# rojas-diego/tokengeex

Measured on AMD Instinct MI355X. Metric: MB/s raw bytes encoded (and tokens/s) at 32K/64K vocab, 1/2/4/8 GPUs, higher is better.
Workload: dtype f64

## Files before the change

### tokengeex_amd/csrc/encode2.hip

```cpp
#include <hip/hip_runtime.h>
#include <stdint.h>

#include "device_common.h"
#include "kernels.h"
#include "trace_body.h"

namespace tgx {

constexpr uint32_t kNoStep2 = 0xFFu;
constexpr uint32_t kRows2Bytes = 64u * 32u * 8u;
constexpr uint64_t kHiHalf = 0xFFFFFFFF00000000ULL;

template <int U>
__device__ __forceinline__ void relax2_step(double sv, double& acc, uint32_t& bpv, uint32_t& fin, uint32_t& fhi) {
    constexpr uint64_t MU = (1ULL << U) | (1ULL << (32 + U));
    fin = sel_u32(MU, bpv, fin);
    fhi = sel_u32(MU, (uint32_t)((uint64_t)__double_as_longlong(acc) >> 32), fhi);
    const double b0 = readlane_f64(acc, (uint32_t)U), b1 = readlane_f64(acc, 32u + (uint32_t)U);
    const double best = sel_f64(kHiHalf, b1, b0);
    const double cand = best + sv;
    const uint64_t take = __builtin_amdgcn_fcmp(cand, acc, 2 ) | MU;
    acc = sel_f64(take, cand, acc);
    bpv = sel_imm_u32<U>(take, bpv);
}
// ... 104 lines not shown
            relax2_step<1>(sv[1], acc, bpv, fin, fhi);
            relax2_step<2>(sv[2], acc, bpv, fin, fhi);
            relax2_step<3>(sv[3], acc, bpv, fin, fhi);
            relax2_step<4>(sv[4], acc, bpv, fin, fhi);
            relax2_step<5>(sv[5], acc, bpv, fin, fhi);
            relax2_step<6>(sv[6], acc, bpv, fin, fhi);
            relax2_step<7>(sv[7], acc, bpv, fin, fhi);
            relax2_step<8>(sv[8], acc, bpv, fin, fhi);
            relax2_step<9>(sv[9], acc, bpv, fin, fhi);
            relax2_step<10>(sv[10], acc, bpv, fin, fhi);
            relax2_step<11>(sv[11], acc, bpv, fin, fhi);
            relax2_step<12>(sv[12], acc, bpv, fin, fhi);
            relax2_step<13>(sv[13], acc, bpv, fin, fhi);
            relax2_step<14>(sv[14], acc, bpv, fin, fhi);
            relax2_step<15>(sv[15], acc, bpv, fin, fhi);
#pragma unroll
            for (int u = 0; u < 16; ++u) sv[u] = scr[(u + 16) * 32];
            relax2_step<16>(sv[0], acc, bpv, fin, fhi);
            relax2_step<17>(sv[1], acc, bpv, fin, fhi);
            relax2_step<18>(sv[2], acc, bpv, fin, fhi);
            relax2_step<19>(sv[3], acc, bpv, fin, fhi);
            relax2_step<20>(sv[4], acc, bpv, fin, fhi);
            relax2_step<21>(sv[5], acc, bpv, fin, fhi);
            relax2_step<22>(sv[6], acc, bpv, fin, fhi);
            relax2_step<23>(sv[7], acc, bpv, fin, fhi);
            relax2_step<24>(sv[8], acc, bpv, fin, fhi);
            relax2_step<25>(sv[9], acc, bpv, fin, fhi);
            relax2_step<26>(sv[10], acc, bpv, fin, fhi);
            relax2_step<27>(sv[11], acc, bpv, fin, fhi);
            relax2_step<28>(sv[12], acc, bpv, fin, fhi);
            relax2_step<29>(sv[13], acc, bpv, fin, fhi);
            relax2_step<30>(sv[14], acc, bpv, fin, fhi);
            relax2_step<31>(sv[15], acc, bpv, fin, fhi);
        }
        __builtin_amdgcn_wave_barrier();
        const bool reached = fhi != 0xFFF00000u;

        if (live && pg >= 1u && pg <= n) {
            const uint8_t b = reached ? (uint8_t)((l - fin - 1u) & 31u) : (uint8_t)0xFF;
            __builtin_nontemporal_store(b, P.bp8 + bp8_base(beg, s) + (PERM ? bp8_perm(pg - 1u) : pg - 1u));
        }
        if (live) {
            const uint32_t left = n - p0;
            if (left < 32u) {
                if (left == l) P.status[s] = (n == 0u || reached) ? 1u : 0u;
                need_new = true;
            } else {
                p0 += 32u;
            }
        }
    }
}

template <bool PERM, bool CARRY, int K>
__global__ __launch_bounds__(256) void trace32_kernel(EncodeParams P) {
    __shared__ typename TraceRingEntry<CARRY>::type ring_all[4][kTraceRing];
    trace_body<32, PERM, false, CARRY, K>(P, ring_all[threadIdx.x >> 6]);
}

hipError_t launch_encode2(const EncodeParams& p, uint32_t num_cus, bool permuted, hipStream_t stream) {
    const uint32_t waves = 5, bpc = 2;
    const uint64_t want = (p.n_samples + 2 * waves - 1) / (2 * waves);
    const uint32_t blocks = (uint32_t)(want < (uint64_t)num_cus * bpc ? (want ? want : 1) : (uint64_t)num_cus * bpc);
    auto fn = p.dropout > 0.0 ? (permuted ? encode2_kernel<true, true> : encode2_kernel<true, false>)
                              : (permuted ? encode2_kernel<false, true> : encode2_kernel<false, false>);
    hipError_t e = hipFuncSetAttribute(reinterpret_cast<const void*>(fn), hipFuncAttributeMaxDynamicSharedMemorySize, 160 * 1024);
    if (e != hipSuccess) return e;
    hipLaunchKernelGGL(fn, dim3(blocks), dim3(64u * waves), waves * kRows2Bytes, stream, p);
    return hipGetLastError();
}
template <bool PERM, bool CARRY>
static void launch_trace32_stride(const EncodeParams& p, uint32_t blocks, hipStream_t stream) {
    switch (p.trace_stride) {
        case 1: hipLaunchKernelGGL((trace32_kernel<PERM, CARRY, 1>), dim3(blocks), dim3(256), 0, stream, p); break;
        case 2: hipLaunchKernelGGL((trace32_kernel<PERM, CARRY, 2>), dim3(blocks), dim3(256), 0, stream, p); break;
        case 3: hipLaunchKernelGGL((trace32_kernel<PERM, CARRY, 3>), dim3(blocks), dim3(256), 0, stream, p); break;
        default: hipLaunchKernelGGL((trace32_kernel<PERM, CARRY, 0>), dim3(blocks), dim3(256), 0, stream, p); break;
    }
}
hipError_t launch_trace32(const EncodeParams& p, uint32_t blocks, bool permuted, hipStream_t stream) {
    if (permuted) {
        if (p.trace_carry) launch_trace32_stride<true, true>(p, blocks, stream);
        else launch_trace32_stride<true, false>(p, blocks, stream);
    } else {
        if (p.trace_carry) launch_trace32_stride<false, true>(p, blocks, stream);
        else launch_trace32_stride<false, false>(p, blocks, stream);
    }
    return hipGetLastError();
}

}
```

### tokengeex_amd/csrc/encode_pass.cpp

```cpp
#include <hip/hip_runtime.h>

#include <algorithm>
#include <chrono>
#include <condition_variable>
#include <cstdio>
#include <cstdlib>
#include <cstring>
#include <mutex>
#include <numeric>
#include <string>
#include <thread>
#include <vector>

#include "../../include/tgx.h"
#include "api_internal.h"
#include "device_internal.h"
#include "pass_internal.h"
#include "kernels.h"
#include "encode_split.h"
#include "ids_in_place.h"
#include "trie_build.h"

using namespace tgx::host;
using namespace tgx::dev;
// ... 46 lines not shown
    std::vector<double> v2((size_t)nv + 1), w2(wvalues.size());
    v2[0] = values[0];
    if (!w2.empty()) w2[0] = wvalues[0];
    unsigned long long total = 0, run = 0;
    for (uint32_t r = 0; r < nv; r++) total += cnt[order[r]];
    std::vector<double> cov((size_t)nv + 1, 0.0);
    for (uint32_t r = 0; r < nv; r++) {
        perm[order[r]] = r + 1u;
        v2[r + 1u] = values[order[r]];
        if (!w2.empty()) w2[r + 1u] = wvalues[order[r]];
        run += cnt[order[r]];
        cov[r + 1u] = total ? (double)run / (double)total : 1.0;
    }
    cov[nv] = 1.0;
    ok = hipMemcpyAsync(d_perm, perm.data(), ((size_t)nv + 1) * 4, hipMemcpyHostToDevice, m->stream) == hipSuccess &&
         tgx::launch_rank_remap(m->d_trie8, (uint32_t)m->flat.table.size(), d_perm, m->stream) == hipSuccess &&
         hipMemcpyAsync(m->d_values, v2.data(), ((size_t)nv + 1) * 8, hipMemcpyHostToDevice, m->stream) == hipSuccess &&
         (w2.empty() || hipMemcpyAsync(m->d_wvalues, w2.data(), ((size_t)nv + 1) * 8, hipMemcpyHostToDevice, m->stream) == hipSuccess) &&
         hipStreamSynchronize(m->stream) == hipSuccess;
    if (!ok) return fail(TGX_ERR_DEVICE, "value re-rank failed: %s", hipGetErrorString(hipGetLastError()));
    m->value_coverage = std::move(cov);
    hp.mark("re-rank");
    return pass.done();
}

}

namespace tgx::dev {

tgx::EncodeParams base_encode_params(const tgx_model* m, const tgx_corpus* c, uint64_t seed) {
    tgx::EncodeParams p{};
    p.text = c->d_text;
    p.offs = c->d_offs;
    p.order = c->d_order;
    p.n_samples = c->n_samples;
    p.trie = m->d_trie;
    p.tokid = m->d_tokid;
    p.root_base = m->flat.table[0].base & ~tgx::kTerminalBit;
    p.lm = m->lm;
    p.n_slots = (uint32_t)m->flat.table.size();
    p.bp = c->d_bp;
    p.tmp = c->d_tmp;
    p.counts = c->d_counts;
    p.status = c->d_status;
    p.bp8 = reinterpret_cast<uint8_t*>(c->d_bp.get());
    p.tokhash = m->d_tokhash;
    p.tokhash_mask = m->tokhash.mask;
    p.tokhash_seed = m->tokhash.seed;
    p.err_sample = &m->d_ctrl->err;
    p.queue = &m->d_ctrl->queue;
    p.seed = seed;
    p.trace_carry = (c->n_samples && c->n_bytes / c->n_samples < 2048) ? 1u : 0u;
    p.trace_stride = tgx::kTraceStride;
    return p;
}

tgx_status check_no_path(tgx_model* m, const tgx_corpus* c) {
    unsigned long long bad = m->h_ctrl->err;
    if (bad == ~0ULL) return TGX_OK;
    if (bad & tgx::kErrCorruptBp)
        return fail(TGX_ERR_DEVICE, "internal error: corrupt back-pointer (sample or text byte %llu)",
                    (unsigned long long)(bad & ~tgx::kErrCorruptBp));
    if (bad & tgx::kErrCountMismatch)
        return fail(TGX_ERR_DEVICE, "internal error: the token count of sample %llu differs between the relaxation and the trace",
                    (unsigned long long)(bad & ~tgx::kErrCountMismatch));
    uint64_t n = c->h_offs[bad + 1] - c->h_offs[bad];
    set_error_detail(bad, n, n);
    return fail(TGX_ERR_NO_PATH, "no path to position %llu/%llu", (unsigned long long)n,
                (unsigned long long)n);
}

}

namespace {

tgx_status redo_long_matches(tgx_model* m, tgx_corpus* c, const tgx::EncodeParams& p) {
    unsigned long long n_redo = 0;
    HIP_TRY(hipMemcpyAsync(&n_redo, &m->d_ctrl->encode_redo, 8, hipMemcpyDeviceToHost, m->stream));
    HIP_TRY(hipStreamSynchronize(m->stream));
    if (n_redo > c->n_samples) return fail(TGX_ERR_DEVICE, "redo list longer than the batch");
    m->last_redo_samples = n_redo;
    if (n_redo) {
        tgx::EncodeParams q = p;
        q.order = c->d_counts;
        q.n_samples = n_redo;
        HIP_TRY(hipMemsetAsync(&m->d_ctrl->queue, 0x00, 8, m->stream));
        time_begin(m, "encode2_kernel");
        HIP_TRY(tgx::launch_encode2(q, (uint32_t)m->num_cus, true, m->stream));
        time_end(m);
    }
    return TGX_OK;
}

tgx_status scan_ids_offsets(tgx_model* m, tgx_corpus* c, tgx_result* r, const char* what, bool with_err);

struct Encode6Choice {
    int e6_bpc;
    uint32_t n_hot6;
    uint32_t pool6;
    bool cold6;
    bool e6_usable;
};
Encode6Choice choose_encode6(const tgx_model* m) {
    int e6_bpc = 2;
    if (const char* e = knob("TGX_E6_BPC")) e6_bpc = std::min(4, std::max(1, atoi(e)));
    uint32_t n_hot6 = std::min(m->n_values, tgx::encode6_max_hot(160u * 1024u / (uint32_t)e6_bpc, 0u));
// ... 102 lines not shown
    if (const char* e = long_tokens ? nullptr : knob("TGX_PPL")) {
        const int v = atoi(e);
        if (v >= 1 && v <= 4) {
            ppl = v;
            bpc = ppl >= 3 ? 1 : 2;
        }
    }
    knob_int("TGX_BPC", 1, 8, &bpc);
    const uint32_t budget = 160u * 1024u / (uint32_t)bpc;
    bool cold = false;
    int per_simd = 0;
    HIP_TRY(tgx::encode5_waves_per_simd(dropout > 0.0, false, ppl, long_tokens, compact, lean, step_ok, want_count, &per_simd));
    int waves = std::min(16, (per_simd / bpc) * 4);
    if ((ppl == 4 || ppl == 3) && bpc == 1 && hot_waves > 0) waves = std::min(waves, hot_waves);
    if (m->n_values > tgx::encode5_max_hot(long_tokens, waves, ppl, budget)) {
        cold = true;
        HIP_TRY(tgx::encode5_waves_per_simd(dropout > 0.0, true, ppl, long_tokens, compact, lean, step_ok, want_count, &per_simd));
        waves = std::min(16, (per_simd / bpc) * 4);
    }
    if (balance_waves > 0 && ppl == 4 && bpc == 1) waves = std::min(waves, balance_waves);
    waves = waves_for_units(waves, rest_n, (uint64_t)cus5 * bpc);
    knob_int("TGX_WAVES", 1, 16, &waves);
    while (waves > 1 && tgx::encode5_max_hot(long_tokens, waves, ppl, budget) < 16u) waves--;
    uint32_t n_hot = std::min(m->n_values, tgx::encode5_max_hot(long_tokens, waves, ppl, budget));
    n_hot = knob_cap_hot("TGX_E5_HOT", n_hot);
    cold = n_hot < m->n_values;
    iq.build_counts = tgx::encode5_counts(dropout > 0.0, cold, ppl, long_tokens);
    const bool in_place = want_count && tgx::ids_in_place(iq);
    const uint64_t rows_per_block = 4 * (uint64_t)waves;
    const uint32_t blocks5 = (uint32_t)std::max<uint64_t>(
        1, std::min<uint64_t>((rest_n + rows_per_block - 1) / rows_per_block, (uint64_t)cus5 * bpc));
    *out = Encode5Geometry{ppl, bpc, waves, per_simd, cold, n_hot, blocks5, compact, lean, step_ok, in_place};
    return TGX_OK;
}

tgx_status trace_rows5(tgx_model* m, tgx_corpus* c, tgx::EncodeParams& p, bool long_tokens, bool in_place, Pass& pass, tgx_result* r) {
    const uint32_t blocks_t = trace_blocks(m, c->n_samples);
    if (in_place) {
        const tgx_status st = scan_ids_offsets(m, c, r, "encode", false);
        if (st != TGX_OK) return st;
        time_begin(m, "trace_kernel");
        HIP_TRY(tgx::launch_trace_in_place(p, tgx::TraceInPlace{r->d_offs, r->d_ids}, blocks_t, m->stream));
        time_end(m);
        m->last_ids_in_place = true;
        return TGX_OK;
    }
    Stamps stamps_t;
    if (!long_tokens) stamps_t = stamps_begin(m, pass, '2', (size_t)blocks_t * 4);
    p.stamps = stamps_t.d;
    time_begin(m, long_tokens ? "trace32_kernel" : "trace_kernel");
    if (long_tokens) HIP_TRY(tgx::launch_trace32(p, blocks_t, true, m->stream));
    else HIP_TRY(tgx::launch_trace(p, blocks_t, m->stream));
    time_end(m);
    if (stamps_t.d) stamps_report(m, stamps_t, 0, "trace stamps", "window", {"setup", "loads", "hops", "append+lookups", "-"});
    p.stamps = nullptr;
    return TGX_OK;
}

tgx_status encode_rows5(tgx_model* m, tgx_corpus* c, tgx::EncodeParams& p, bool long_tokens, Pass& pass, tgx_result* r) {
    tgx_status st = ensure_value_ranks(m, c);
    if (st != TGX_OK) return st;
    m->last_redo_samples = 0;
    const Encode6Choice e6 = choose_encode6(m);
    tgx::EncodeSplit split;
    if (c->n_samples && !long_tokens && e6.e6_usable) split = split_long_samples(m, c, e6);
    const uint64_t n_long = split.n_long;
    const uint32_t corun_cus = split.corun_cus;
    Encode5Geometry g;
    if ((st = choose_encode5(m, c, p, long_tokens, n_long, corun_cus, r != nullptr, &g)) != TGX_OK) return st;
    m->last_n_hot = g.n_hot;
    if (!g.in_place) {
        if ((st = ensure_scratch(c, true)) != TGX_OK) return st;
        p.tmp = c->d_tmp;
    }
    const uint64_t rest_n = c->n_samples - n_long;
    m->last_lean_items = !g.lean ? 0u : ((rest_n ? (uint32_t)tgx::encode5_lean_items(g.cold, g.ppl, g.step_ok) : 0u) |
                                         (n_long ? (uint32_t)tgx::encode6_lean_items() << 8 : 0u));
    m->last_encode_waves_per_cu = std::min(g.bpc, g.per_simd / ((g.waves + 3) / 4)) * g.waves;
    tgx::Encode5Params q{};
    q.trie8 = m->d_trie8;
    q.trie_bytes = (uint32_t)(m->flat.table.size() * sizeof(tgx::Trie8Rec));
    q.values = m->d_values;
    q.root_base = m->root_base8;
    q.n_values = m->n_values;
    q.n_hot = g.n_hot;
    q.claim_chunk = claim_chunk_for(c->n_bytes, c->n_samples);
    if (const char* e = knob("TGX_CLAIM_CHUNK")) q.claim_chunk = (uint32_t)std::min(64, std::max(1, atoi(e)));
    m->last_long_samples = n_long;
    m->last_corun_cus = n_long ? corun_cus : 0u;
    tgx::EncodeParams p6 = p;
    tgx::Encode5Params q6 = q;
    uint32_t blocks6 = 0;
    if (n_long) {
        p6.n_samples = n_long;
        blocks6 = (uint32_t)std::min<uint64_t>((n_long + 3) / 4, (uint64_t)(corun_cus ? (int)corun_cus : m->num_cus) * (uint64_t)e6.e6_bpc);
        q6.n_hot = e6.n_hot6;
        q6.pool = e6.cold6 ? e6.pool6 : 0u;
        if (!corun_cus) {
            time_begin(m, "encode6_kernel");
            HIP_TRY(tgx::launch_encode6(p6, q6, e6.cold6, g.lean, blocks6, m->stream));
            time_end(m);
            HIP_TRY(hipMemsetAsync(&m->d_ctrl->queue, 0x00, 8, m->stream));
        } else {
            if (!m->stream2) {
                HIP_TRY(hipStreamCreateWithFlags(&m->stream2, hipStreamNonBlocking));
                HIP_TRY(hipEventCreateWithFlags(&m->ev_fork, hipEventDisableTiming));
                HIP_TRY(hipEventCreateWithFlags(&m->ev_join, hipEventDisableTiming));
// ... 113 lines not shown
    p.stamps = stamps4.d;
    time_begin(m, "encode4_kernel");
    HIP_TRY(tgx::launch_encode4(p, ppl, waves, blocks4, root, m->stream));
    time_end(m);
    if (stamps4.d) stamps_report(m, stamps4, 0, "stamps", "iteration", {"switch", "text", "walk", "relax", "store"});
    p.stamps = nullptr;
    p.order = c->d_order;
    p.n_samples = c->n_samples;
    time_begin(m, "trace_kernel");
    HIP_TRY(tgx::launch_trace(p, trace_blocks(m, c->n_samples), m->stream));
    time_end(m);
    return TGX_OK;
}

tgx_status encode_rows2(tgx_model* m, tgx_corpus* c, tgx::EncodeParams& p, bool rows2) {
    m->last_redo_samples = 0;
    if (!rows2) {
        p.redo_count = &m->d_ctrl->encode_redo;
        p.redo_list = c->d_counts;
        HIP_TRY(hipMemsetAsync(&m->d_ctrl->encode_redo, 0x00, 8, m->stream));
        time_begin(m, "encode4l_kernel");
        HIP_TRY(tgx::launch_encode4l(p, (uint32_t)m->num_cus, m->stream));
        time_end(m);
        const tgx_status rst = redo_long_matches(m, c, p);
        if (rst != TGX_OK) return rst;
    } else {
        time_begin(m, "encode2_kernel");
        HIP_TRY(tgx::launch_encode2(p, (uint32_t)m->num_cus, false, m->stream));
        time_end(m);
    }
    time_begin(m, "trace32_kernel");
    HIP_TRY(tgx::launch_trace32(p, trace_blocks(m, c->n_samples), !rows2, m->stream));
    time_end(m);
    return TGX_OK;
}

tgx_status encode_fused(tgx_model* m, tgx_corpus* c, const tgx::EncodeParams& p) {
    time_begin(m, "encode_kernel");
    HIP_TRY(tgx::launch_encode(p, grid_blocks(m, c->n_samples), m->stream));
    time_end(m);
    return TGX_OK;
}

tgx_status run_encode_kernel(tgx_model* m, tgx_corpus* c, double dropout, uint64_t seed, Pass& pass, tgx_result* r) {
    m->last_ids_in_place = false;
    tgx_status st = ensure_scratch(c, false);
    if (st != TGX_OK) return st;
    HIP_TRY(hipMemsetAsync(&m->d_ctrl->queue, 0x00, 8, m->stream));
    HIP_TRY(hipMemsetAsync(&m->d_ctrl->err, 0xFF, 8, m->stream));
    tgx::EncodeParams p = base_encode_params(m, c, seed);
    p.dropout = dropout;
    if (const char* e = knob("TGX_TRACE_CARRY")) p.trace_carry = atoi(e) ? 1u : 0u;
    if (const char* e = knob("TGX_TRACE_STRIDE")) p.trace_stride = (uint32_t)std::min(3, std::max(0, atoi(e)));
    p.flags = debug_flags();
    const char* force = knob("TGX_PATH");
    const bool use4 = m->lm <= 16 && m->scores_finite && m->d_tokhash && !(force && strcmp(force, "fused") == 0);
    const bool use2 = !use4 && m->lm <= 32 && m->scores_finite && m->d_tokhash && !(force && strcmp(force, "fused") == 0);
    const bool long_tokens = m->lm > 16;
    const bool use5 = (use4 || use2) && m->have_trie8 &&
                      !(force && (strcmp(force, "rows4") == 0 || strcmp(force, "rows2") == 0 || strcmp(force, "rows4l") == 0));
    if (debug_on())
        fprintf(stderr, "[tgx] encode: S=%llu N=%llu lm=%u path=%s slots=%zu root_base=%u values=%u\n",
                (unsigned long long)c->n_samples, (unsigned long long)c->n_bytes, p.lm, use4 ? (use5 ? "rows5" : "rows4") : (use2 ? "rows2" : "fused"),
                m->flat.table.size(), p.root_base, m->n_values);
    m->last_lean_items = 0;
    if (use5) return encode_rows5(m, c, p, long_tokens, pass, r);
    if ((st = ensure_scratch(c, true)) != TGX_OK) return st;
    p.tmp = c->d_tmp;
    if (use4) return encode_rows4(m, c, p, pass);
    if (use2) return encode_rows2(m, c, p, force && strcmp(force, "rows2") == 0);
    return encode_fused(m, c, p);
}

tgx_status scan_ids_offsets(tgx_model* m, tgx_corpus* c, tgx_result* r, const char* what, bool with_err) {
    const uint64_t S = c->n_samples;
    if (!c->d_scan_tmp) {
        if (tgx::scan_temp_bytes(S, &c->scan_tmp_bytes) != hipSuccess) return fail(TGX_ERR_DEVICE, "scan temp-size query failed");
        if (c->scan_tmp_bytes && c->d_scan_tmp.alloc(m->device, c->scan_tmp_bytes) != hipSuccess)
            return fail(TGX_ERR_DEVICE, "out of device memory (scan)");
    }
    time_begin(m, "scan_counts_kernel");
    if (tgx::launch_scan(c->d_counts, r->d_offs, S, c->d_scan_tmp, c->scan_tmp_bytes, m->stream) != hipSuccess)
        return fail(TGX_ERR_DEVICE, "scan launch failed");
    time_end(m);
    if ((with_err && hipMemcpyAsync(&m->h_ctrl->err, &m->d_ctrl->err, 8, hipMemcpyDeviceToHost, m->stream) != hipSuccess) ||
        hipMemcpyAsync(&m->h_ctrl->total_tokens, r->d_offs + S, 8, hipMemcpyDeviceToHost, m->stream) != hipSuccess ||
        hipStreamSynchronize(m->stream) != hipSuccess)
        return fail(TGX_ERR_DEVICE, "%s pass failed: %s", what, hipGetErrorString(hipGetLastError()));
    if (with_err) {
        const tgx_status st = check_no_path(m, c);
        if (st != TGX_OK) return st;
    }
    r->n_tokens = m->h_ctrl->total_tokens;
    if (r->n_tokens > c->n_bytes) return fail(TGX_ERR_DEVICE, "internal error: %s pass counted more tokens than bytes", what);
    if (r->d_ids.alloc(m->device, (size_t)r->n_tokens * 4 + 256) != hipSuccess)
        return fail(TGX_ERR_DEVICE, "out of device memory (result ids)");
    return TGX_OK;
}

}

tgx_status tgx::dev::compact_ids(tgx_model* m, tgx_corpus* c, tgx_result* r, const char* what) {
    const uint64_t S = c->n_samples;
    const tgx_status sst = scan_ids_offsets(m, c, r, what, true);
    if (sst != TGX_OK) return sst;
    tgx::CompactParams cp{};
// ... 346 lines not shown
```

### tokengeex_amd/csrc/kernels.h

```cpp
#pragma once
#include <hip/hip_runtime.h>
#include <stdint.h>

#include "decode.h"
#include "fim.h"
#include "spans.h"

namespace tgx {

constexpr uint32_t kTraceStride = 2;

struct EncodeParams {
    const uint8_t* text;
    const uint64_t* offs;
    const uint32_t* order;
    uint64_t n_samples;
    const void* trie;
    const uint32_t* tokid;
    uint32_t root_base;
    uint32_t n_slots;
    uint32_t lm;
    uint32_t* bp;
    uint32_t* tmp;
    uint32_t* counts;
    uint32_t* status;
    uint8_t* bp8;
    const void* tokhash;
    uint32_t tokhash_mask;
    uint32_t tokhash_seed;
    unsigned long long* err_sample;
    unsigned long long* queue;
    unsigned long long* redo_count;
    uint32_t* redo_list;
    double dropout;
    uint64_t seed;
    uint32_t flags;
    unsigned long long* stamps;
    uint32_t trace_carry;
    uint32_t trace_stride;
};

struct Encode5Params {
    const void* trie8;
    uint32_t trie_bytes;
    const double* values;
    uint32_t root_base;
    uint32_t n_values;
    uint32_t n_hot;
    uint32_t claim_chunk;
    uint32_t list_off, root_off, idx_off;
    uint32_t ctrl_off, ring_off, ring_slots;
    uint32_t pool;
    unsigned int* started;
};

struct CompactParams {
    const uint64_t* offs;
    const uint32_t* order;
    uint64_t n_samples;
    const uint32_t* tmp;
    const uint64_t* out_offs;
    uint32_t* ids;
};

struct EstepParams {
    const uint8_t* text;
    const uint64_t* offs;
    const uint32_t* order;
    uint64_t n_samples;
    const void* trie_fwd;
    const void* trie_rev;
    uint32_t root_fwd, root_rev;
    uint32_t lm;
    uint64_t snippet_len;
    double* alpha;
    double* expected_slot;
    uint32_t n_slots_rev, n_replicas;
    double* logz_sum;
    unsigned long long* err_sample;
    double dropout;
    uint64_t seed;
};

hipError_t launch_pair_keys(const uint32_t* ids, const uint64_t* out_offs, uint64_t n_samples, uint32_t shift,
                            unsigned long long sentinel, unsigned long long* keys, uint32_t blocks, hipStream_t stream);
hipError_t pair_sort_temp_bytes(uint64_t n, size_t* bytes);
hipError_t pair_sort(void* temp, size_t temp_bytes, const unsigned long long* in, unsigned long long* out,
                     uint64_t n, unsigned int end_bit, hipStream_t stream);
hipError_t pair_rle_temp_bytes(uint64_t n, size_t* bytes);
// ... 330 lines not shown
```

### tokengeex_amd/csrc/kernels.hip

```cpp
#include <hip/hip_runtime.h>
#include <stdint.h>

#include <rocprim/device/device_scan.hpp>
#include <rocprim/iterator/transform_iterator.hpp>

#include "kernels.h"
#include "trace_body.h"
#include "device_common.h"

namespace tgx {

struct WaveCtx {
    const uint4* __restrict__ trie;
    uint32_t root_base;
    double dropout;
    uint64_t seed;
    bool use_dropout;
    uint32_t flags;
};

__device__ __forceinline__ void block_generic(const WaveCtx& C, const uint8_t* __restrict__ text, uint32_t n,
                                              uint32_t s, uint32_t p0, uint32_t lane, uint32_t LM,
                                              double* sc, uint32_t* hl, uint8_t* txt, uint32_t* __restrict__ bp,
                                              double& acc, uint32_t& bpv, uint64_t& reach, uint32_t& reach_n) {
// ... 424 lines not shown
            relax5_step<6>(sv[6], acc, bpv, fin[g], fhi);
            relax5_step<7>(sv[7], acc, bpv, fin[g], fhi);
            relax5_step<8>(sv[8], acc, bpv, fin[g], fhi);
            relax5_step<9>(sv[9], acc, bpv, fin[g], fhi);
            relax5_step<10>(sv[10], acc, bpv, fin[g], fhi);
            relax5_step<11>(sv[11], acc, bpv, fin[g], fhi);
            relax5_step<12>(sv[12], acc, bpv, fin[g], fhi);
            relax5_step<13>(sv[13], acc, bpv, fin[g], fhi);
            relax5_step<14>(sv[14], acc, bpv, fin[g], fhi);
            relax5_step<15>(sv[15], acc, bpv, fin[g], fhi);
            reached[g] = fhi != 0xFFF00000u;
        }
        __builtin_amdgcn_wave_barrier();
        TGX_STAMP(3)

        uint8_t* const bpw = P.bp8 + bp8_base(beg, s);
#pragma unroll
        for (int g = 0; g < PPL; ++g)
            if (live && pg[g] >= 1u && pg[g] <= n) {
                const uint32_t b = reached[g] ? ((l - fin[g] - 1u) & 15u) : 0xFFu;
                const uint32_t j = pg[g] - 1u, kq = (j >> 4) & 3u;
                pk = (kq == 0u) ? b : (pk | (b << (8u * kq)));
                pk_j = j;
                pk_dirty = true;
                if (kq == 3u) {
                    __builtin_nontemporal_store(pk, reinterpret_cast<uint32_t*>(bpw + (bp8_perm(j) & ~3u)));
                    pk_dirty = false;
                }
            }
        if (live && n - p0 < SPAN && pk_dirty) {
            __builtin_nontemporal_store(pk, reinterpret_cast<uint32_t*>(bpw + (bp8_perm(pk_j) & ~3u)));
            pk_dirty = false;
        }
        if (live) {
            const uint32_t left = n - p0;
            if (left < SPAN) {
#pragma unroll
                for (int g = 0; g < PPL; ++g)
                    if (left == 16u * g + l) P.status[s] = (n == 0u || reached[g]) ? 1u : 0u;
                need_new = true;
            } else {
                p0 += SPAN;
            }
        }
        TGX_STAMP(4)
    }
    if (STAMP && lane == 0 && P.stamps) {
        unsigned long long* o = P.stamps + (size_t)(blockIdx.x * wpb + wave) * 8u;
        for (int i = 0; i < 5; ++i) o[i] = seg[i];
        o[5] = iters;
    }
}

template <bool STAMP, bool CARRY, int K, bool INPLACE = false>
__global__ __launch_bounds__(256, INPLACE ? 8 : 1) void trace_kernel(EncodeParams P, TraceInPlace O) {
    static_assert(!(STAMP && INPLACE), "the stamped build writes through tmp");
    __shared__ typename TraceRingEntry<CARRY>::type ring_all[4][kTraceRing];
    trace_body<16, true, STAMP, CARRY, K, INPLACE>(P, ring_all[threadIdx.x >> 6], O);
}

__global__ __launch_bounds__(1024) void scan_counts_kernel(const uint32_t* __restrict__ counts,
                                                           uint64_t* __restrict__ offsets,
                                                           uint64_t n) {
    __shared__ uint64_t wsum[16];
    __shared__ uint64_t carry_s;
    constexpr uint32_t E = 8;
    const uint32_t tid = threadIdx.x, lane = tid & 63u, wave = tid >> 6;
    if (tid == 0) carry_s = 0;
    __syncthreads();
    for (uint64_t base = 0; base < n; base += 1024u * E) {
        const uint64_t i0 = base + (uint64_t)tid * E;
        uint32_t c[E];
        uint64_t v = 0;
#pragma unroll
        for (uint32_t e = 0; e < E; ++e) {
            c[e] = (i0 + e < n) ? counts[i0 + e] : 0u;
            v += c[e];
        }
        uint64_t x = v;
        for (int off = 1; off < 64; off <<= 1) {
            uint64_t y = __shfl_up(x, off);
            if ((int)lane >= off) x += y;
        }
        if (lane == 63) wsum[wave] = x;
        __syncthreads();
        uint64_t wprefix = 0;
        for (uint32_t w = 0; w < wave; ++w) wprefix += wsum[w];
        const uint64_t carry = carry_s;
        uint64_t run = carry + wprefix + x - v;
#pragma unroll
        for (uint32_t e = 0; e < E; ++e) {
            if (i0 + e < n) offsets[i0 + e] = run;
            run += c[e];
        }
        __syncthreads();
        if (tid == 1023) carry_s = run;
        __syncthreads();
    }
    if (tid == 0) offsets[n] = carry_s;
}

template <bool ROWS>
__global__ __launch_bounds__(256) void compact_kernel(CompactParams P) {
    const uint32_t lane = threadIdx.x & 63u;
    const uint32_t sub = ROWS ? (lane & 15u) : lane, width = ROWS ? 16u : 64u;
    const uint64_t n_units = (uint64_t)gridDim.x * 4u * (ROWS ? 4u : 1u);
    const uint32_t wave_id = blockIdx.x * 4u + (threadIdx.x >> 6);
    for (uint64_t k = ROWS ? (uint64_t)wave_id * 4u + (lane >> 4) : (uint64_t)wave_id; k < P.n_samples; k += n_units) {
        const uint32_t s = ROWS ? (uint32_t)k : P.order[k];
        const uint64_t end = P.offs[s + 1];
        const uint64_t o0 = P.out_offs[s];
// ... 29 lines not shown
    if (t == 16) return encode_kernel<16>;
    if (t == 32) return encode_kernel<32>;
    return encode_kernel<0>;
}

hipError_t launch_encode(const EncodeParams& p, uint32_t blocks, hipStream_t stream) {
    const uint32_t lds = encode_lds_bytes_per_block(p.lm);
    const dim3 block(64u * encode_waves_per_block(p.lm));
    hipLaunchKernelGGL(pick_kernel(p.lm), dim3(blocks), block, lds, stream, p);
    return hipGetLastError();
}

hipError_t encode_max_blocks_per_cu(uint32_t lm, int* out) {
    const uint32_t lds = encode_lds_bytes_per_block(lm);
    const int threads = (int)(64u * encode_waves_per_block(lm));
    if (lds > 160u * 1024u) return hipErrorInvalidValue;
    encode_fn fn = pick_kernel(lm);
    hipError_t e = hipFuncSetAttribute(reinterpret_cast<const void*>(fn),
                                       hipFuncAttributeMaxDynamicSharedMemorySize, (int)lds);
    if (e != hipSuccess) return e;
    return hipOccupancyMaxActiveBlocksPerMultiprocessor(out, fn, threads, lds);
}

typedef void (*encode4_fn)(EncodeParams);
static encode4_fn pick_encode4(bool dropout, int ppl, bool stamp, bool root) {
    if (stamp) return encode4_kernel<false, 1, true, false>;
    if (root) return dropout ? encode4_kernel<true, 1, false, true> : encode4_kernel<false, 1, false, true>;
    if (ppl == 1) return dropout ? encode4_kernel<true, 1, false, false> : encode4_kernel<false, 1, false, false>;
    if (ppl == 2) return dropout ? encode4_kernel<true, 2, false, false> : encode4_kernel<false, 2, false, false>;
    return dropout ? encode4_kernel<true, 4, false, false> : encode4_kernel<false, 4, false, false>;
}
uint32_t encode4_group_bytes() { return kRows4GroupBytes; }
uint32_t encode4_lds_bytes(int waves, int ppl, bool root) {
    return (root ? 4096u : 0u) + (uint32_t)waves * (uint32_t)ppl * kRows4GroupBytes;
}
hipError_t encode4_waves_per_simd(bool dropout, int ppl, bool root, int* out) {
    root = root && ppl == 1;
    hipFuncAttributes attr;
    hipError_t e = hipFuncGetAttributes(&attr, reinterpret_cast<const void*>(pick_encode4(dropout, ppl, false, root)));
    if (e != hipSuccess) return e;
    const int regs = (attr.numRegs + 7) & ~7;
    *out = regs > 0 ? (512 / regs > 8 ? 8 : 512 / regs) : 8;
    return hipSuccess;
}
hipError_t launch_encode4(const EncodeParams& p, int ppl, int waves, uint32_t blocks, bool root, hipStream_t stream) {
    const bool stamp = p.stamps != nullptr;
    root = root && !stamp && ppl == 1;
    encode4_fn fn = pick_encode4(p.dropout > 0.0, ppl, stamp, root);
    hipError_t e = hipFuncSetAttribute(reinterpret_cast<const void*>(fn), hipFuncAttributeMaxDynamicSharedMemorySize, 160 * 1024);
    if (e != hipSuccess) return e;
    hipLaunchKernelGGL(fn, dim3(blocks), dim3(64u * (uint32_t)waves), encode4_lds_bytes(waves, stamp ? 1 : ppl, root), stream, p);
    return hipGetLastError();
}
template <bool STAMP, bool CARRY>
static void launch_trace_stride(const EncodeParams& p, uint32_t blocks, hipStream_t stream) {
    switch (p.trace_stride) {
        case 1: hipLaunchKernelGGL((trace_kernel<STAMP, CARRY, 1>), dim3(blocks), dim3(256), 0, stream, p, TraceInPlace{nullptr, nullptr}); break;
        case 2: hipLaunchKernelGGL((trace_kernel<STAMP, CARRY, 2>), dim3(blocks), dim3(256), 0, stream, p, TraceInPlace{nullptr, nullptr}); break;
        case 3: hipLaunchKernelGGL((trace_kernel<STAMP, CARRY, 3>), dim3(blocks), dim3(256), 0, stream, p, TraceInPlace{nullptr, nullptr}); break;
        default: hipLaunchKernelGGL((trace_kernel<STAMP, CARRY, 0>), dim3(blocks), dim3(256), 0, stream, p, TraceInPlace{nullptr, nullptr}); break;
    }
}
hipError_t launch_trace(const EncodeParams& p, uint32_t blocks, hipStream_t stream) {
    if (p.stamps)
        launch_trace_stride<true, false>(p, blocks, stream);
    else if (p.trace_carry)
        launch_trace_stride<false, true>(p, blocks, stream);
    else
        launch_trace_stride<false, false>(p, blocks, stream);
    return hipGetLastError();
}

template <bool CARRY>
static void launch_trace_in_place_stride(const EncodeParams& p, const TraceInPlace& o, uint32_t blocks, hipStream_t stream) {
    switch (p.trace_stride) {
        case 1: hipLaunchKernelGGL((trace_kernel<false, CARRY, 1, true>), dim3(blocks), dim3(256), 0, stream, p, o); break;
        case 2: hipLaunchKernelGGL((trace_kernel<false, CARRY, 2, true>), dim3(blocks), dim3(256), 0, stream, p, o); break;
        case 3: hipLaunchKernelGGL((trace_kernel<false, CARRY, 3, true>), dim3(blocks), dim3(256), 0, stream, p, o); break;
        default: hipLaunchKernelGGL((trace_kernel<false, CARRY, 0, true>), dim3(blocks), dim3(256), 0, stream, p, o); break;
    }
}
hipError_t launch_trace_in_place(const EncodeParams& p, const TraceInPlace& o, uint32_t blocks, hipStream_t stream) {
    if (p.stamps || !o.out_offs || !o.ids) return hipErrorInvalidValue;
    if (p.trace_carry)
        launch_trace_in_place_stride<true>(p, o, blocks, stream);
    else
        launch_trace_in_place_stride<false>(p, o, blocks, stream);
    return hipGetLastError();
}

struct WidenU32 {
    __host__ __device__ uint64_t operator()(uint32_t x) const { return (uint64_t)x; }
};
hipError_t scan_temp_bytes(uint64_t n, size_t* bytes) {
    *bytes = 0;
    if (n <= 65536) return hipSuccess;
    auto in = rocprim::make_transform_iterator((const uint32_t*)nullptr, WidenU32());
    return rocprim::exclusive_scan(nullptr, *bytes, in, (uint64_t*)nullptr, (uint64_t)0, (size_t)(n + 1), rocprim::plus<uint64_t>());
}
hipError_t launch_scan(uint32_t* counts, uint64_t* offsets, uint64_t n, void* temp, size_t temp_bytes, hipStream_t stream) {
    if (n <= 65536 || !temp) {
        hipLaunchKernelGGL(scan_counts_kernel, dim3(1), dim3(1024), 0, stream, counts, offsets, n);
        return hipGetLastError();
    }
    hipError_t e = hipMemsetAsync(counts + n, 0, 4, stream);
    if (e != hipSuccess) return e;
    auto in = rocprim::make_transform_iterator((const uint32_t*)counts, WidenU32());
    return rocprim::exclusive_scan(temp, temp_bytes, in, offsets, (uint64_t)0, (size_t)(n + 1), rocprim::plus<uint64_t>(), stream);
}

hipError_t launch_compact(const CompactParams& p, uint32_t blocks, bool rows, hipStream_t stream) {
    if (rows)
        hipLaunchKernelGGL(compact_kernel<true>, dim3(blocks), dim3(256), 0, stream, p);
    else
        hipLaunchKernelGGL(compact_kernel<false>, dim3(blocks), dim3(256), 0, stream, p);
    return hipGetLastError();
}

}
```

### tokengeex_amd/csrc/trace_body.h

```cpp
#pragma once
#include <hip/hip_runtime.h>
#include <stdint.h>

#include "device_common.h"
#include "kernels.h"

namespace tgx {

constexpr uint32_t kTraceRing = 128;

#define TGX_TRACE_STAMP(i)                                             \
    if (STAMP) {                                                       \
        __builtin_amdgcn_sched_barrier(0);                             \
        const uint64_t _now = (uint64_t)__builtin_amdgcn_s_memtime(); \
        __builtin_amdgcn_s_waitcnt(0xC07F);                            \
        __builtin_amdgcn_sched_barrier(0);                             \
        seg[i] += _now - t_last;                                       \
        t_last = _now;                                                 \
    }

__device__ __forceinline__ int32_t trace_lane_addr(int32_t p) {
    return (p < 0 ? 0 : p) << 2;
}
__device__ __forceinline__ int32_t trace_square(int32_t p) {
    const int32_t got = __builtin_amdgcn_ds_bpermute(trace_lane_addr(p), p);
    return p < 0 ? p : got;
}
template <int K>
__device__ __forceinline__ uint64_t trace_hops(uint32_t prev, int32_t& qq) {
    static_assert(K >= 0 && K <= 3, "strides of 1, 2, 4, 8 tokens");
    if constexpr (K == 0) {
        uint64_t ends = 0;
        while (qq >= 0) {
            asm("s_bitset1_b64 %0, %1" : "+s"(ends) : "s"(qq));
            qq = (int32_t)readlane_u32(prev, (uint32_t)qq);
        }
        return ends;
    } else {
        int32_t p[K + 1];
        p[0] = (int32_t)prev;
#pragma unroll
        for (int k = 1; k <= K; ++k) p[k] = trace_square(p[k - 1]);
        uint64_t visited = 0;
        while (qq >= 0) {
            asm("s_bitset1_b64 %0, %1" : "+s"(visited) : "s"(qq));
            qq = (int32_t)readlane_u32((uint32_t)p[K], (uint32_t)qq);
        }
        uint64_t on = visited;
#pragma unroll
        for (int k = K - 1; k >= 0; --k) {
            const bool send = __builtin_amdgcn_inverse_ballot_w64(on) && p[k] >= 0;
            const int32_t got = __builtin_amdgcn_ds_permute(send ? trace_lane_addr(p[k]) : 63 << 2, 1);
            on |= __builtin_amdgcn_ballot_w64(got != 0) & ~(1ULL << 63);
        }
        return on;
    }
}

template <bool CARRY> struct TraceRingEntry { using type = uint2; };
template <> struct TraceRingEntry<true> { using type = uint4; };
template <uint32_t LM, bool PERM, bool STAMP, bool CARRY, int K, bool INPLACE = false>
__device__ __forceinline__ void trace_body(const EncodeParams& P, typename TraceRingEntry<CARRY>::type* ring, const TraceInPlace O = TraceInPlace{nullptr, nullptr}) {
    static_assert(LM == 16 || LM == 32, "token lengths of up to 16 or 32 bytes");
    constexpr uint32_t LMASK = LM - 1u;
    constexpr int NW = (int)LM / 4;
    const uint32_t lane = threadIdx.x & 63u;
    const uint32_t wpb = blockDim.x >> 6;
    const uint32_t n_waves = gridDim.x * wpb;
    const uint32_t wave_id = (uint32_t)__builtin_amdgcn_readfirstlane((int)(blockIdx.x * wpb + (threadIdx.x >> 6)));
    const uint4* __restrict__ table = reinterpret_cast<const uint4*>(P.tokhash);
    uint64_t seg[6] = {0, 0, 0, 0, 0, 0};
    uint64_t t_last = STAMP ? (uint64_t)__builtin_amdgcn_s_memtime() : 0;
    uint32_t iters = 0;
    const uint64_t n_rounds = (P.n_samples + n_waves - 1) / n_waves;
    constexpr uint32_t kNone = 0xFFFFFFFFu;
    auto sample_of_round = [&](uint64_t rnd) -> uint32_t {
        const uint64_t k = rnd * n_waves + ((rnd & 1u) ? (uint64_t)(n_waves - 1u - wave_id) : (uint64_t)wave_id);
        return (rnd < n_rounds && k < P.n_samples) ? P.order[k] : kNone;
    };
    struct MetaRaw {
        uint64_t beg, end;
        uint32_t reach;
        uint64_t out_end;
        uint32_t count;
    };
    struct Meta {
        uint32_t s;
        uint64_t beg;
        uint32_t n, reach_n;
        uint64_t out_end;
        uint32_t count;
    };
    auto meta_request = [&](uint32_t smp) -> MetaRaw {
        MetaRaw r{0, 0, 1u, 0, 0u};
        if (smp != kNone) {
            r.beg = P.offs[smp];
            r.end = P.offs[smp + 1];
            r.reach = P.status[smp];
            if constexpr (INPLACE) {
                r.out_end = O.out_offs[smp + 1];
                r.count = P.counts[smp];
            }
        }
        return r;
    };
    auto meta_read = [&](uint32_t smp, const MetaRaw& r) -> Meta {
        Meta mt{smp, 0, 0, 1u, 0, 0u};
        if (smp != kNone) {
            mt.beg = first_u64(r.beg);
            mt.n = (uint32_t)(first_u64(r.end) - mt.beg);
            mt.reach_n = (mt.n == 0) ? 1u : (uint32_t)__builtin_amdgcn_readfirstlane((int)r.reach);
            if constexpr (INPLACE) {
                mt.out_end = first_u64(r.out_end);
                mt.count = (uint32_t)__builtin_amdgcn_readfirstlane((int)r.count);
            }
        }
        return mt;
    };
    auto first_window = [&](const Meta& mt) -> uint32_t {
        if (mt.s == kNone || mt.n == 0 || !mt.reach_n || (P.flags & 4u)) return 0u;
        const uint8_t* __restrict__ bpn = P.bp8 + bp8_base(mt.beg, mt.s);
        const uint32_t wq0 = (mt.n - 1u) & ~63u;
        return (wq0 + lane < mt.n) ? (uint32_t)bpn[PERM ? bp8_perm(wq0 + lane) : wq0 + lane] : 0u;
    };
    uint32_t head = 0, fill = 0;
    uint64_t flush_beg = 0, flush_out_top = 0;
    auto lookup = [&](uint32_t m) {
        if (lane < m && !(P.flags & 16u)) {
            const auto e = ring[(head + lane) & (kTraceRing - 1u)];
            uint32_t len;
            uint64_t end, out;
            if constexpr (CARRY) {
                len = e.y >> 16;
                end = ((uint64_t)(e.y & 0xFFFFu) << 32) | e.x;
                out = ((uint64_t)e.w << 32) | e.z;
            } else {
                len = e.y;
                end = flush_beg + e.x;
                out = flush_out_top - 1u - lane;
            }
            struct __attribute__((packed, aligned(1))) Bytes16 { uint32_t w[4]; };
            const Bytes16* __restrict__ src = reinterpret_cast<const Bytes16*>(P.text + (end - len));
            uint32_t b[8] = {0, 0, 0, 0, 0, 0, 0, 0};
#pragma unroll
            for (int j = 0; j < NW; j += 4) {
                const Bytes16 raw = src[j / 4];
#pragma unroll
                for (int i = 0; i < 4; ++i) {
                    const uint32_t nb = len > 4u * (j + i) ? len - 4u * (j + i) : 0u;
                    b[j + i] = nb >= 4u ? raw.w[i] : (raw.w[i] & ((1u << (8u * nb)) - 1u));
                }
            }
            const uint64_t hk = LM == 16 ? tok_hash64_dev(b[0], b[1], b[2], b[3], len, P.tokhash_seed)
                                         : tok_hash64_long_dev(b, len, P.tokhash_seed);
            uint32_t slot = (uint32_t)hk & P.tokhash_mask;
            uint32_t id = 0;
            bool found = false;
            for (uint32_t probe = 0; probe <= P.tokhash_mask && !found; ++probe) {
                const uint4 t = load_rec(table, slot);
                if (t.w == 0u) break;
                if (t.x == (uint32_t)hk && t.y == (uint32_t)(hk >> 32)) {
                    id = t.z;
                    found = true;
                }
                slot = (slot + 1u) & P.tokhash_mask;
            }
            if (!found) atomicMin(P.err_sample, (unsigned long long)((end - len) & ((1ULL << 62) - 1ULL)) | (1ULL << 62));
            if constexpr (INPLACE) O.ids[out] = id;
            else P.tmp[out] = id;
        }
        if constexpr (!CARRY) flush_out_top -= m;
        head = (head + m) & (kTraceRing - 1u);
        fill -= m;
    };
    Meta cur;
    {
        const uint32_t s0 = (uint32_t)__builtin_amdgcn_readfirstlane((int)sample_of_round(0));
        cur = meta_read(s0, meta_request(s0));
    }
    uint32_t s_next_raw = sample_of_round(1);
    uint32_t h_first = first_window(cur);
    for (uint64_t rnd = 0; rnd < n_rounds; ++rnd) {
        const uint32_t s_next = (uint32_t)__builtin_amdgcn_readfirstlane((int)s_next_raw);
        const uint32_t s_after_raw = sample_of_round(rnd + 2);
        const MetaRaw nxt_raw = meta_request(s_next);
        const uint32_t s = cur.s;
        const uint64_t beg = cur.beg;
        const uint32_t n = cur.n;
        const uint32_t reach_n = cur.reach_n;
        const bool have = s != kNone;
        const uint8_t* __restrict__ bp = P.bp8 + (have ? bp8_base(beg, s) : 0);
        uint32_t total = INPLACE ? cur.count : 0u;
        uint64_t out_top = INPLACE ? cur.out_end : beg + n;
        flush_beg = beg;
        flush_out_top = out_top;
        int64_t q = (have && reach_n) ? (int64_t)n - 1 : (int64_t)-1;
        if (P.flags & 4u) q = -1;

        uint32_t h_cur = h_first;
        TGX_TRACE_STAMP(0)
        while (q >= 0) {
            iters++;
            const uint32_t wq = (uint32_t)q & ~63u;
            const uint32_t idx = wq + lane;
            const uint32_t h = h_cur;
            uint32_t prev = lane - ((h & LMASK) + 1u);
            asm volatile("" : "+v"(prev) : : "memory");
            uint32_t h_next = 0;
            if (wq >= 64u) h_next = (uint32_t)bp[PERM ? bp8_perm(wq - 64u + lane) : wq - 64u + lane];
            TGX_TRACE_STAMP(1)
            int32_t qq = (int32_t)((uint32_t)q - wq);
            uint64_t ends = trace_hops<K>(prev, qq);
            q = (int64_t)wq + qq;
            uint32_t cnt = (uint32_t)__popcll(ends);
            if constexpr (INPLACE) {
                const bool ov = cnt > total;
                ends = ov ? 0ULL : ends;
                cnt = ov ? 0u : cnt;
                q = ov ? (int64_t)-1 : q;
                total = ov ? 0xFFFFFFFFu : total;
            }
            TGX_TRACE_STAMP(2)
            if ((ends >> lane) & 1ULL) {
                const uint32_t below = __builtin_amdgcn_mbcnt_hi((uint32_t)(ends >> 32), __builtin_amdgcn_mbcnt_lo((uint32_t)ends, 0u));
                if constexpr (CARRY) {
                    const uint64_t end = beg + idx + 1u, out = out_top - 1u - (cnt - 1u - below);
                    ring[(head + fill + (cnt - 1u - below)) & (kTraceRing - 1u)] =
                        make_uint4((uint32_t)end, (uint32_t)(end >> 32) | (((h & LMASK) + 1u) << 16), (uint32_t)out, (uint32_t)(out >> 32));
                } else {
                    ring[(head + fill + (cnt - 1u - below)) & (kTraceRing - 1u)] = make_uint2(idx + 1u, (h & LMASK) + 1u);
                }
            }
            fill += cnt;
            if constexpr (INPLACE) total -= cnt;
            else total += cnt;
            out_top -= cnt;
            __builtin_amdgcn_wave_barrier();
            if (fill >= 64u) lookup(64u);
            TGX_TRACE_STAMP(3)
            h_cur = h_next;
        }
        const Meta nxt = meta_read(s_next, nxt_raw);
        h_first = first_window(nxt);
        if constexpr (!CARRY) {
            if (fill) lookup(fill);
        }
        if (have && lane == 0) {
            if constexpr (INPLACE) {
                if (total != 0u) atomicMin(P.err_sample, kErrCountMismatch | (unsigned long long)s);
            } else {
                P.counts[s] = total;
            }
            if (!reach_n) atomicMin(P.err_sample, (unsigned long long)s);
        }
        cur = nxt;
        s_next_raw = s_after_raw;
    }
    if (fill) lookup(fill);
    if (STAMP && lane == 0 && P.stamps) {
        unsigned long long* o = P.stamps + (size_t)wave_id * 8u;
        for (int i = 0; i < 5; ++i) o[i] = seg[i];
        o[5] = iters;
    }
}

}
```

Baseline: 72500.

## Software-pipeline trace token lookups across text load, hash probe and finish stages

```diff
diff --git a/tokengeex_amd/csrc/encode2.hip b/tokengeex_amd/csrc/encode2.hip
--- a/tokengeex_amd/csrc/encode2.hip
+++ b/tokengeex_amd/csrc/encode2.hip
@@ -180,10 +180,10 @@
     }
 }
 
-template <bool PERM, bool CARRY, int K>
-__global__ __launch_bounds__(256) void trace32_kernel(EncodeParams P) {
+template <bool PERM, bool CARRY, int K, int PIPE = 0>
+__global__ __launch_bounds__(256, PIPE > 0 ? 8 : 1) void trace32_kernel(EncodeParams P) {
     __shared__ typename TraceRingEntry<CARRY>::type ring_all[4][kTraceRing];
-    trace_body<32, PERM, false, CARRY, K>(P, ring_all[threadIdx.x >> 6]);
+    trace_body<32, PERM, false, CARRY, K, false, PIPE>(P, ring_all[threadIdx.x >> 6]);
 }
 
 hipError_t launch_encode2(const EncodeParams& p, uint32_t num_cus, bool permuted, hipStream_t stream) {
@@ -197,22 +197,30 @@
     hipLaunchKernelGGL(fn, dim3(blocks), dim3(64u * waves), waves * kRows2Bytes, stream, p);
     return hipGetLastError();
 }
-template <bool PERM, bool CARRY>
+template <bool PERM, bool CARRY, int PIPE>
 static void launch_trace32_stride(const EncodeParams& p, uint32_t blocks, hipStream_t stream) {
     switch (p.trace_stride) {
-        case 1: hipLaunchKernelGGL((trace32_kernel<PERM, CARRY, 1>), dim3(blocks), dim3(256), 0, stream, p); break;
-        case 2: hipLaunchKernelGGL((trace32_kernel<PERM, CARRY, 2>), dim3(blocks), dim3(256), 0, stream, p); break;
-        case 3: hipLaunchKernelGGL((trace32_kernel<PERM, CARRY, 3>), dim3(blocks), dim3(256), 0, stream, p); break;
-        default: hipLaunchKernelGGL((trace32_kernel<PERM, CARRY, 0>), dim3(blocks), dim3(256), 0, stream, p); break;
+        case 1: hipLaunchKernelGGL((trace32_kernel<PERM, CARRY, 1, PIPE>), dim3(blocks), dim3(256), 0, stream, p); break;
+        case 2: hipLaunchKernelGGL((trace32_kernel<PERM, CARRY, 2, PIPE>), dim3(blocks), dim3(256), 0, stream, p); break;
+        case 3: hipLaunchKernelGGL((trace32_kernel<PERM, CARRY, 3, PIPE>), dim3(blocks), dim3(256), 0, stream, p); break;
+        default: hipLaunchKernelGGL((trace32_kernel<PERM, CARRY, 0, PIPE>), dim3(blocks), dim3(256), 0, stream, p); break;
+    }
+}
+template <bool PERM, bool CARRY>
+static void launch_trace32_pipe(const EncodeParams& p, uint32_t blocks, hipStream_t stream) {
+    switch (p.trace_pipe) {
+        case 1: launch_trace32_stride<PERM, CARRY, 1>(p, blocks, stream); break;
+        case 2: launch_trace32_stride<PERM, CARRY, 2>(p, blocks, stream); break;
+        default: launch_trace32_stride<PERM, CARRY, 0>(p, blocks, stream); break;
     }
 }
 hipError_t launch_trace32(const EncodeParams& p, uint32_t blocks, bool permuted, hipStream_t stream) {
     if (permuted) {
-        if (p.trace_carry) launch_trace32_stride<true, true>(p, blocks, stream);
-        else launch_trace32_stride<true, false>(p, blocks, stream);
+        if (p.trace_carry) launch_trace32_pipe<true, true>(p, blocks, stream);
+        else launch_trace32_pipe<true, false>(p, blocks, stream);
     } else {
-        if (p.trace_carry) launch_trace32_stride<false, true>(p, blocks, stream);
-        else launch_trace32_stride<false, false>(p, blocks, stream);
+        if (p.trace_carry) launch_trace32_pipe<false, true>(p, blocks, stream);
+        else launch_trace32_pipe<false, false>(p, blocks, stream);
     }
     return hipGetLastError();
 }
diff --git a/tokengeex_amd/csrc/encode_pass.cpp b/tokengeex_amd/csrc/encode_pass.cpp
--- a/tokengeex_amd/csrc/encode_pass.cpp
+++ b/tokengeex_amd/csrc/encode_pass.cpp
@@ -122,6 +122,7 @@
     p.seed = seed;
     p.trace_carry = (c->n_samples && c->n_bytes / c->n_samples < 2048) ? 1u : 0u;
     p.trace_stride = tgx::kTraceStride;
+    p.trace_pipe = m->lm > 16 ? tgx::kTrace32Pipe : tgx::kTracePipe;
     return p;
 }
 
@@ -330,7 +331,7 @@
     if (long_tokens) HIP_TRY(tgx::launch_trace32(p, blocks_t, true, m->stream));
     else HIP_TRY(tgx::launch_trace(p, blocks_t, m->stream));
     time_end(m);
-    if (stamps_t.d) stamps_report(m, stamps_t, 0, "trace stamps", "window", {"setup", "loads", "hops", "append+lookups", "-"});
+    if (stamps_t.d) stamps_report(m, stamps_t, 0, "trace stamps", "window", {"setup", "loads", "hops", "append+lookups", "staged-lookups"});
     p.stamps = nullptr;
     return TGX_OK;
 }
@@ -550,6 +551,7 @@
     p.dropout = dropout;
     if (const char* e = knob("TGX_TRACE_CARRY")) p.trace_carry = atoi(e) ? 1u : 0u;
     if (const char* e = knob("TGX_TRACE_STRIDE")) p.trace_stride = (uint32_t)std::min(3, std::max(0, atoi(e)));
+    if (const char* e = knob("TGX_TRACE_PIPE")) p.trace_pipe = (uint32_t)std::min(2, std::max(0, atoi(e)));
     p.flags = debug_flags();
     const char* force = knob("TGX_PATH");
     const bool use4 = m->lm <= 16 && m->scores_finite && m->d_tokhash && !(force && strcmp(force, "fused") == 0);
diff --git a/tokengeex_amd/csrc/kernels.h b/tokengeex_amd/csrc/kernels.h
--- a/tokengeex_amd/csrc/kernels.h
+++ b/tokengeex_amd/csrc/kernels.h
@@ -9,6 +9,8 @@
 namespace tgx {
 
 constexpr uint32_t kTraceStride = 2;
+constexpr uint32_t kTracePipe = 2;
+constexpr uint32_t kTrace32Pipe = 0;
 
 struct EncodeParams {
     const uint8_t* text;
@@ -35,6 +37,7 @@
     double dropout;
     uint64_t seed;
     uint32_t flags;
+    uint32_t trace_pipe;
     unsigned long long* stamps;
     uint32_t trace_carry;
     uint32_t trace_stride;
diff --git a/tokengeex_amd/csrc/kernels.hip b/tokengeex_amd/csrc/kernels.hip
--- a/tokengeex_amd/csrc/kernels.hip
+++ b/tokengeex_amd/csrc/kernels.hip
@@ -500,11 +500,11 @@
     }
 }
 
-template <bool STAMP, bool CARRY, int K, bool INPLACE = false>
-__global__ __launch_bounds__(256, INPLACE ? 8 : 1) void trace_kernel(EncodeParams P, TraceInPlace O) {
+template <bool STAMP, bool CARRY, int K, bool INPLACE = false, int PIPE = 0>
+__global__ __launch_bounds__(256, (INPLACE || PIPE > 0) ? 8 : 1) void trace_kernel(EncodeParams P, TraceInPlace O) {
     static_assert(!(STAMP && INPLACE), "the stamped build writes through tmp");
     __shared__ typename TraceRingEntry<CARRY>::type ring_all[4][kTraceRing];
-    trace_body<16, true, STAMP, CARRY, K, INPLACE>(P, ring_all[threadIdx.x >> 6], O);
+    trace_body<16, true, STAMP, CARRY, K, INPLACE, PIPE>(P, ring_all[threadIdx.x >> 6], O);
 }
 
 __global__ __launch_bounds__(1024) void scan_counts_kernel(const uint32_t* __restrict__ counts,
@@ -640,40 +640,40 @@
     hipLaunchKernelGGL(fn, dim3(blocks), dim3(64u * (uint32_t)waves), encode4_lds_bytes(waves, stamp ? 1 : ppl, root), stream, p);
     return hipGetLastError();
 }
-template <bool STAMP, bool CARRY>
-static void launch_trace_stride(const EncodeParams& p, uint32_t blocks, hipStream_t stream) {
+template <bool STAMP, bool CARRY, bool INPLACE, int PIPE>
+static void launch_trace_stride(const EncodeParams& p, const TraceInPlace& o, uint32_t blocks, hipStream_t stream) {
     switch (p.trace_stride) {
-        case 1: hipLaunchKernelGGL((trace_kernel<STAMP, CARRY, 1>), dim3(blocks), dim3(256), 0, stream, p, TraceInPlace{nullptr, nullptr}); break;
-        case 2: hipLaunchKernelGGL((trace_kernel<STAMP, CARRY, 2>), dim3(blocks), dim3(256), 0, stream, p, TraceInPlace{nullptr, nullptr}); break;
-        case 3: hipLaunchKernelGGL((trace_kernel<STAMP, CARRY, 3>), dim3(blocks), dim3(256), 0, stream, p, TraceInPlace{nullptr, nullptr}); break;
-        default: hipLaunchKernelGGL((trace_kernel<STAMP, CARRY, 0>), dim3(blocks), dim3(256), 0, stream, p, TraceInPlace{nullptr, nullptr}); break;
+        case 1: hipLaunchKernelGGL((trace_kernel<STAMP, CARRY, 1, INPLACE, PIPE>), dim3(blocks), dim3(256), 0, stream, p, o); break;
+        case 2: hipLaunchKernelGGL((trace_kernel<STAMP, CARRY, 2, INPLACE, PIPE>), dim3(blocks), dim3(256), 0, stream, p, o); break;
+        case 3: hipLaunchKernelGGL((trace_kernel<STAMP, CARRY, 3, INPLACE, PIPE>), dim3(blocks), dim3(256), 0, stream, p, o); break;
+        default: hipLaunchKernelGGL((trace_kernel<STAMP, CARRY, 0, INPLACE, PIPE>), dim3(blocks), dim3(256), 0, stream, p, o); break;
+    }
+}
+template <bool STAMP, bool CARRY, bool INPLACE>
+static void launch_trace_pipe(const EncodeParams& p, const TraceInPlace& o, uint32_t blocks, hipStream_t stream) {
+    switch (p.trace_pipe) {
+        case 1: launch_trace_stride<STAMP, CARRY, INPLACE, 1>(p, o, blocks, stream); break;
+        case 2: launch_trace_stride<STAMP, CARRY, INPLACE, 2>(p, o, blocks, stream); break;
+        default: launch_trace_stride<STAMP, CARRY, INPLACE, 0>(p, o, blocks, stream); break;
     }
 }
 hipError_t launch_trace(const EncodeParams& p, uint32_t blocks, hipStream_t stream) {
+    const TraceInPlace none{nullptr, nullptr};
     if (p.stamps)
-        launch_trace_stride<true, false>(p, blocks, stream);
+        launch_trace_pipe<true, false, false>(p, none, blocks, stream);
     else if (p.trace_carry)
-        launch_trace_stride<false, true>(p, blocks, stream);
+        launch_trace_pipe<false, true, false>(p, none, blocks, stream);
     else
-        launch_trace_stride<false, false>(p, blocks, stream);
+        launch_trace_pipe<false, false, false>(p, none, blocks, stream);
     return hipGetLastError();
 }
 
-template <bool CARRY>
-static void launch_trace_in_place_stride(const EncodeParams& p, const TraceInPlace& o, uint32_t blocks, hipStream_t stream) {
-    switch (p.trace_stride) {
-        case 1: hipLaunchKernelGGL((trace_kernel<false, CARRY, 1, true>), dim3(blocks), dim3(256), 0, stream, p, o); break;
-        case 2: hipLaunchKernelGGL((trace_kernel<false, CARRY, 2, true>), dim3(blocks), dim3(256), 0, stream, p, o); break;
-        case 3: hipLaunchKernelGGL((trace_kernel<false, CARRY, 3, true>), dim3(blocks), dim3(256), 0, stream, p, o); break;
-        default: hipLaunchKernelGGL((trace_kernel<false, CARRY, 0, true>), dim3(blocks), dim3(256), 0, stream, p, o); break;
-    }
-}
 hipError_t launch_trace_in_place(const EncodeParams& p, const TraceInPlace& o, uint32_t blocks, hipStream_t stream) {
     if (p.stamps || !o.out_offs || !o.ids) return hipErrorInvalidValue;
     if (p.trace_carry)
-        launch_trace_in_place_stride<true>(p, o, blocks, stream);
+        launch_trace_pipe<false, true, true>(p, o, blocks, stream);
     else
-        launch_trace_in_place_stride<false>(p, o, blocks, stream);
+        launch_trace_pipe<false, false, true>(p, o, blocks, stream);
     return hipGetLastError();
 }
 
diff --git a/tokengeex_amd/csrc/trace_body.h b/tokengeex_amd/csrc/trace_body.h
--- a/tokengeex_amd/csrc/trace_body.h
+++ b/tokengeex_amd/csrc/trace_body.h
@@ -59,7 +59,15 @@
 
 template <bool CARRY> struct TraceRingEntry { using type = uint2; };
 template <> struct TraceRingEntry<true> { using type = uint4; };
-template <uint32_t LM, bool PERM, bool STAMP, bool CARRY, int K, bool INPLACE = false>
+template <int PIPE, int NW> struct TraceStages {
+    uint32_t a_raw[NW] = {}, a_len = 0;
+    uint64_t a_out = 0, a_pos = 0;
+    uint4 b_rec = {0u, 0u, 0u, 0u};
+    uint64_t b_hk = 0, b_out = 0, b_pos = 0;
+    uint32_t b_live = 0;
+};
+template <int NW> struct TraceStages<0, NW> {};
+template <uint32_t LM, bool PERM, bool STAMP, bool CARRY, int K, bool INPLACE = false, int PIPE = 0>
 __device__ __forceinline__ void trace_body(const EncodeParams& P, typename TraceRingEntry<CARRY>::type* ring, const TraceInPlace O = TraceInPlace{nullptr, nullptr}) {
     static_assert(LM == 16 || LM == 32, "token lengths of up to 16 or 32 bytes");
     constexpr uint32_t LMASK = LM - 1u;
@@ -125,8 +133,85 @@
     };
     uint32_t head = 0, fill = 0;
     uint64_t flush_beg = 0, flush_out_top = 0;
+    TraceStages<PIPE, NW> st;
     auto lookup = [&](uint32_t m) {
-        if (lane < m && !(P.flags & 16u)) {
+        if constexpr (PIPE > 0) {
+            auto& a_raw = st.a_raw;
+            uint32_t &a_len = st.a_len, &b_live = st.b_live;
+            uint64_t &a_out = st.a_out, &a_pos = st.a_pos, &b_hk = st.b_hk, &b_out = st.b_out, &b_pos = st.b_pos;
+            uint4& b_rec = st.b_rec;
+            auto finish = [&]() {
+                if (b_live) {
+                    uint4 t = b_rec;
+                    uint32_t slot = (uint32_t)b_hk & P.tokhash_mask, id = 0;
+                    bool found = false;
+                    for (uint32_t probe = 0;;) {
+                        if (t.w == 0u) break;
+                        if (t.x == (uint32_t)b_hk && t.y == (uint32_t)(b_hk >> 32)) {
+                            id = t.z;
+                            found = true;
+                            break;
+                        }
+                        slot = (slot + 1u) & P.tokhash_mask;
+                        if (++probe > P.tokhash_mask) break;
+                        t = load_rec(table, slot);
+                    }
+                    if (!found) atomicMin(P.err_sample, (unsigned long long)(b_pos & ((1ULL << 62) - 1ULL)) | (1ULL << 62));
+                    if constexpr (INPLACE) O.ids[b_out] = id;
+                    else P.tmp[b_out] = id;
+                }
+            };
+            auto probe_first = [&]() {
+                b_live = a_len;
+                if (a_len) {
+                    uint32_t b[8] = {0, 0, 0, 0, 0, 0, 0, 0};
+#pragma unroll
+                    for (int j = 0; j < NW; ++j) {
+                        const uint32_t nb = a_len > 4u * j ? a_len - 4u * j : 0u;
+                        b[j] = nb >= 4u ? a_raw[j] : (a_raw[j] & ((1u << (8u * nb)) - 1u));
+                    }
+                    b_hk = LM == 16 ? tok_hash64_dev(b[0], b[1], b[2], b[3], a_len, P.tokhash_seed)
+                                    : tok_hash64_long_dev(b, a_len, P.tokhash_seed);
+                    if constexpr (PIPE == 1) b_rec = load_rec(table, (uint32_t)b_hk & P.tokhash_mask);
+                    else b_rec = table[(uint32_t)b_hk & P.tokhash_mask];
+                    b_out = a_out;
+                    b_pos = a_pos;
+                }
+            };
+            auto issue = [&]() {
+                a_len = 0;
+                if (lane < m && !(P.flags & 16u)) {
+                    const auto e = ring[(head + lane) & (kTraceRing - 1u)];
+                    uint64_t end;
+                    if constexpr (CARRY) {
+                        a_len = e.y >> 16;
+                        end = ((uint64_t)(e.y & 0xFFFFu) << 32) | e.x;
+                        a_out = ((uint64_t)e.w << 32) | e.z;
+                    } else {
+                        a_len = e.y;
+                        end = flush_beg + e.x;
+                        a_out = flush_out_top - 1u - lane;
+                    }
+                    a_pos = end - a_len;
+                    struct __attribute__((packed, aligned(1))) Bytes16 { uint32_t w[4]; };
+                    const Bytes16* __restrict__ src = reinterpret_cast<const Bytes16*>(P.text + a_pos);
+#pragma unroll
+                    for (int j = 0; j < NW; j += 4) {
+                        const Bytes16 raw = src[j / 4];
+#pragma unroll
+                        for (int i = 0; i < 4; ++i) a_raw[j + i] = raw.w[i];
+                    }
+                }
+            };
+            if constexpr (PIPE == 1) {
+                probe_first();
+                finish();
+            } else {
+                finish();
+                probe_first();
+            }
+            issue();
+        } else if (lane < m && !(P.flags & 16u)) {
             const auto e = ring[(head + lane) & (kTraceRing - 1u)];
             uint32_t len;
             uint64_t end, out;
@@ -209,6 +294,10 @@
             uint32_t h_next = 0;
             if (wq >= 64u) h_next = (uint32_t)bp[PERM ? bp8_perm(wq - 64u + lane) : wq - 64u + lane];
             TGX_TRACE_STAMP(1)
+            if constexpr (PIPE > 0) {
+                if (fill >= 64u) lookup(64u);
+                TGX_TRACE_STAMP(4)
+            }
             int32_t qq = (int32_t)((uint32_t)q - wq);
             uint64_t ends = trace_hops<K>(prev, qq);
             q = (int64_t)wq + qq;
@@ -236,12 +325,17 @@
             else total += cnt;
             out_top -= cnt;
             __builtin_amdgcn_wave_barrier();
-            if (fill >= 64u) lookup(64u);
+            if constexpr (PIPE == 0) {
+                if (fill >= 64u) lookup(64u);
+            }
             TGX_TRACE_STAMP(3)
             h_cur = h_next;
         }
         const Meta nxt = meta_read(s_next, nxt_raw);
         h_first = first_window(nxt);
+        if constexpr (PIPE > 0) {
+            if (fill >= 64u) lookup(64u);
+        }
         if constexpr (!CARRY) {
             if (fill) lookup(fill);
         }
@@ -257,6 +351,10 @@
         s_next_raw = s_after_raw;
     }
     if (fill) lookup(fill);
+    if constexpr (PIPE > 0) {
+#pragma nounroll
+        for (int i = 0; i < PIPE; ++i) lookup(0u);
+    }
     if (STAMP && lane == 0 && P.stamps) {
         unsigned long long* o = P.stamps + (size_t)wave_id * 8u;
         for (int i = 0; i < 5; ++i) o[i] = seg[i];
```

Result: no change. 73220, median of 6 (+1.0%).
